# EdwardFerdian/4DFlowNet

Hardware: AMD Instinct MI355X
Metric: 3D patches/sec (train step, patch=24, res×2) (higher is better)
Workload: dtype f32; 1 GPU; cfg2 train_step: patch_size=24 res_increase=2 batch=8/GPU low_resblock=8 hi_resblock=4 fp32; global_batch=8, parallelism=dp1, collective=none

## Files before the change

### 4dflownet_amd/_lib.py

```python
import contextlib
import ctypes
import os

from . import build as _build

_HERE = os.path.dirname(os.path.abspath(__file__))
LIB_PATH = os.path.join(_HERE, "lib4dflow_hip.so")
TEST_LIB_PATH = os.path.join(_HERE, "lib4dflow_hip_test.so")

c_fp = ctypes.c_void_p
c_i = ctypes.c_int
c_i64 = ctypes.c_int64
c_f = ctypes.c_float
c_sz = ctypes.c_size_t

SIGNATURES = {
    "fdn_version": (c_i, []),
    "fdn_last_error": (ctypes.c_char_p, []),
    "fdn_input_features": (c_i, [c_fp] * 8 + [c_i64, c_fp]),
    "fdn_pack_conv64_weights": (c_i, [c_fp, c_fp, c_fp, c_fp]),
    "fdn_conv3d_fwd": (c_i, [c_fp] * 7 + [c_i] * 10 + [c_f, c_i, c_fp]),
    "fdn_conv3d_dgrad": (c_i, [c_fp] * 4 + [c_i] * 10 + [c_fp]),
    "fdn_conv_cout1_dgrad_folded": (c_i, [c_fp, c_fp, c_fp, c_i, c_f, c_fp, c_fp, c_fp, c_sz, c_i, c_i, c_i, c_i, c_i, c_i, c_fp]),
    "fdn_conv_cout1_dgrad_folded_mask": (c_i, [c_fp, c_fp, c_fp, c_i, c_f, c_fp, c_fp, c_fp, c_sz, c_i, c_i, c_i, c_i, c_i, c_i, c_fp]),
    "fdn_fold_halo": (c_i, [c_fp, c_fp, c_fp, c_i, c_fp, c_fp, c_i, c_f, c_fp, c_i, c_i, c_i, c_i, c_i, c_fp]),
    "fdn_conv3d_dgrad_fused": (c_i, [c_fp] * 5 + [c_i, c_f, c_fp, c_i, c_i, c_i, c_i, c_i, c_fp]),
    "fdn_conv64_mask_ok": (c_i, [c_i] * 5),
    "fdn_conv64_fwd_mask": (c_i, [c_fp] * 6 + [c_i] * 5 + [c_f, c_i, c_fp]),
    "fdn_conv64_dgrad_fused_mask": (c_i, [c_fp] * 5 + [c_i, c_f, c_fp, c_i, c_i, c_i, c_i, c_i, c_fp]),
    "fdn_conv64_dgrad_fused_multi": (c_i, [c_fp, c_fp, c_i] + [c_fp] * 4 + [c_i, c_f, c_fp, c_i, c_i, c_i, c_i, c_i, c_fp]),
    "fdn_conv3d_dgrad_fused_part": (c_i, [c_fp] * 5 + [c_i, c_f, c_fp, c_i, c_i, c_i, c_i, c_i, c_i, c_fp]),
    "fdn_fold_halo_border": (c_i, [c_fp, c_fp, c_fp, c_i, c_fp, c_fp, c_i, c_f, c_fp, c_i, c_i, c_i, c_i, c_fp]),
    "fdn_conv1x1_dgrad": (c_i, [c_fp] * 6 + [c_i64, c_fp]),
    "fdn_conv3d_wgrad_workspace_bytes": (c_sz, [c_i] * 7),
    "fdn_conv3d_wgrad_batch_workspace_bytes": (c_sz, [c_i] * 5),
    "fdn_conv3d_wgrad_batch": (c_i, [c_fp, c_fp, c_fp, c_fp, c_i, c_fp, c_sz] + [c_i] * 5 + [c_fp]),
    "fdn_conv3d_wgrad": (c_i, [c_fp] * 6 + [c_sz] + [c_i] * 10 + [c_fp]),
    "fdn_upsample_trilinear_fwd": (c_i, [c_fp, c_fp] + [c_i] * 6 + [c_fp]),
    "fdn_upsample_trilinear_bwd": (c_i, [c_fp, c_fp, c_i, c_f, c_fp] + [c_i] * 6 + [c_fp]),
    "fdn_loss_metrics": (c_i, [c_fp] * 8 + [c_i, c_i64, c_fp]),
    "fdn_loss_metrics_div": (c_i, [c_fp] * 5 + [c_f] + [c_fp] * 3 + [c_i] * 4 + [c_fp]),
    "fdn_gather_patches": (c_i, [c_fp, c_fp, c_i, c_i, c_fp]),
    "fdn_l2_sumsq": (c_i, [c_fp, c_fp, c_i64, c_fp, c_fp]),
    "fdn_adam_step": (c_i, [c_fp] * 5 + [c_i64] + [c_f] * 5 + [c_fp, c_fp, c_fp]),
    "fdn_sum_partials": (c_i, [c_fp, c_i, c_fp, c_fp]),
    "fdn_l2_sumsq_partials": (c_i, [c_fp, c_fp, c_i64, c_fp, c_fp]),
    "fdn_pack_conv64_weights_batch": (c_i, [c_fp, c_fp, c_i, c_fp, c_fp]),
    "fdn_conv64_pack_streams": (c_i, [c_i] * 6),
    "fdn_pack_conv64_weights_batch_streams": (c_i, [c_fp, c_fp, c_i, c_fp, c_i, c_i, c_fp]),
    "fdn_pack_conv64_weights_bf16": (c_i, [c_fp, c_fp, c_fp, c_fp]),
    "fdn_pack_conv64_weights_bf16_batch": (c_i, [c_fp, c_fp, c_i, c_fp, c_fp]),
    "fdn_conv64_fwd_bf16": (c_i, [c_fp] * 5 + [c_i] * 5 + [c_f, c_fp]),
    "fdn_conv64_dgrad_fused_bf16": (c_i, [c_fp] * 5 + [c_i, c_f, c_fp, c_i, c_i, c_i, c_i, c_fp]),
    "fdn_conv64_fwd_bf16_mask": (c_i, [c_fp] * 6 + [c_i] * 5 + [c_f, c_fp]),
    "fdn_conv64_dgrad_fused_bf16_mask": (c_i, [c_fp] * 6 + [c_i, c_f, c_fp, c_i, c_i, c_i, c_i, c_fp]),
    "fdn_conv64_dgrad_fused_bf16_multi": (c_i, [c_fp, c_fp, c_i] + [c_fp] * 4 + [c_i, c_f, c_fp, c_i, c_i, c_i, c_i, c_fp]),
    "fdn_fold_halo_border_bf16": (c_i, [c_fp, c_fp, c_fp, c_i, c_fp, c_fp, c_i, c_f, c_fp, c_i, c_i, c_i, c_i, c_fp]),
    "fdn_input_features_bf16": (c_i, [c_fp] * 8 + [c_i64, c_fp]),
    "fdn_conv3d_fwd_bf16": (c_i, [c_fp] * 7 + [c_i] * 10 + [c_f, c_fp]),
    "fdn_conv3d_wgrad_bf16_workspace_bytes": (c_sz, [c_i] * 7),
    "fdn_conv3d_wgrad_bf16": (c_i, [c_fp] * 6 + [c_sz] + [c_i] * 9 + [c_fp]),
    "fdn_conv3d_wgrad_bf16_batch_workspace_bytes": (c_sz, [c_i] * 5),
    "fdn_conv3d_wgrad_bf16_batch": (c_i, [c_fp, c_fp, c_fp, c_fp, c_i, c_fp, c_sz] + [c_i] * 4 + [c_fp]),
    "fdn_conv_cout1_dgrad_folded_bf16": (c_i, [c_fp, c_fp, c_fp, c_i, c_f, c_fp, c_fp, c_fp, c_sz, c_i, c_i, c_i, c_i, c_i, c_i, c_fp]),
    "fdn_conv_cout1_dgrad_folded_bf16_mask": (c_i, [c_fp, c_fp, c_fp, c_fp, c_i, c_f, c_fp, c_fp, c_fp, c_sz, c_i, c_i, c_i, c_i, c_i, c_i, c_fp]),
    "fdn_conv1x1_dgrad_bf16": (c_i, [c_fp] * 6 + [c_i64, c_fp]),
    "fdn_upsample_trilinear_fwd_bf16": (c_i, [c_fp, c_fp] + [c_i] * 6 + [c_fp]),
    "fdn_upsample_trilinear_bwd_bf16": (c_i, [c_fp, c_fp, c_i, c_f, c_fp] + [c_i] * 6 + [c_fp]),
}


DEBUG_SIGNATURES = {
    "fdn_debug_set_conv64_mt": (c_i, [c_i]),
    "fdn_debug_set_conv64_dbg": (c_i, [c_i]),
    "fdn_debug_set_conv64_shell_slabs": (c_i, [c_i]),
    "fdn_debug_set_conv64_wface_direct": (c_i, [c_i]),
    "fdn_debug_set_conv64_split_dgrad": (c_i, [c_i]),
    "fdn_debug_set_conv64_bf16_mt": (c_i, [c_i]),
    "fdn_debug_set_conv64_bf16_dbg": (c_i, [c_i]),
    "fdn_debug_set_conv64_bf16_mode2": (c_i, [c_i]),
    "fdn_debug_set_heads_mfma": (c_i, [c_i]),
    "fdn_debug_set_upsample_bwd_hb": (c_i, [c_i]),
    "fdn_debug_set_wgrad64_direct": (c_i, [c_i]),
    "fdn_debug_set_conv64_wino_dbg": (c_i, [c_i]),
    "fdn_debug_set_conv64_wino_tile": (c_i, [c_i]),
    "fdn_debug_set_conv64_wino2d_dbg": (c_i, [c_i]),
    "fdn_debug_set_conv64_wino2d_tile": (c_i, [c_i]),
    "fdn_debug_set_conv64_wino2d_variant": (c_i, [c_i]),
    "fdn_debug_set_conv64_wino2d_mb": (c_i, [c_i]),
    "fdn_debug_set_cin3_mfma": (c_i, [c_i]),
    "fdn_debug_set_conv1x1_mfma": (c_i, [c_i]),
    "fdn_debug_set_wgrad64_wino_dbg": (c_i, [c_i]),
    "fdn_debug_set_wgrad64_wino_nodep": (c_i, [c_i]),
    "fdn_debug_set_wgrad64_bf16_dbg": (c_i, [c_i]),
    "fdn_debug_set_wgrad64_bf16_variant": (c_i, [c_i]),
    "fdn_debug_plan_log": (c_i, [c_i]),
    "fdn_debug_plan_read": (c_sz, [ctypes.c_char_p, c_sz]),
}


class FdnError(RuntimeError):
    pass


FDN_VERSION = 161


_product = None
_test = None
_lib = None


def _open(path, sigs, test_hooks=False):
    try:
        built = _build.ensure_built(test_hooks=test_hooks)
    except Exception as e:
        raise FdnError("%s is not usable (%s): %s.  Run `python __graft_entry__.py` or `python 4dflownet_amd/build.py`; "
                       "there is no CPU fallback." % (os.path.basename(path), path, e)) from e
    assert os.path.samefile(built, path)
    lib = ctypes.CDLL(path)
    for name, (res, args) in sigs.items():
        fn = getattr(lib, name)
        fn.restype = res
        fn.argtypes = args
    return lib


def _check_version(lib, path):
    have = lib.fdn_version()
    if have != FDN_VERSION:
        raise FdnError("%s reports fdn_version() = %d, this package mirrors include/fdn.h at FDN_VERSION %d: rebuild (python 4dflownet_amd/build.py)"
                       % (os.path.basename(path), have, FDN_VERSION))
    return lib


def load():
    global _lib, _product
    if _lib is not None:
        return _lib
    if _product is None:
        _product = _check_version(_open(LIB_PATH, SIGNATURES), LIB_PATH)
    _lib = _product
    return _lib


@contextlib.contextmanager
def test_build():
    global _lib, _test
    if _test is None:
        sigs = dict(SIGNATURES)
        sigs.update(DEBUG_SIGNATURES)
        _test = _check_version(_open(TEST_LIB_PATH, sigs, test_hooks=True), TEST_LIB_PATH)
    prev = _lib
    _lib = _test
    try:
        yield _test
    finally:
        _lib = prev


def check(rc, what):
    if rc != 0:
        msg = load().fdn_last_error()
        raise FdnError("%s failed (rc=%d): %s" % (what, rc, msg.decode() if msg else "?"))
```

### 4dflownet_amd/csrc/wgrad64_wino.hip

```cpp
#include "fdn_common.h"
#include <type_traits>

namespace {

struct WgWinoArgs {
    const float* x;
    const float* dz;
    float* partial;
    int N, D, H, W;
    int DT;
    int nth, ntw, ntiles, S;
    unsigned bytes;
    int dbg;
};

FDN_HOOK_VAR(int, fdn_wgrad64_wino_dbg, 0);

constexpr int WTH = 6, WTG = 2, WTW = 4 * WTG;
constexpr int GROWB = 1536;
constexpr int VBYTES = (WTH + 2) * WTG * GROWB;
constexpr int ZBYTES = WTH * WTG * GROWB;
constexpr int WBUFB = VBYTES + ZBYTES;
constexpr int kLocSlot = 5, kXSlot = 6, kZSlot = 13;
constexpr int kLocSlotZ = 10;
constexpr int XSCRATCH = 6 * 4096;
constexpr int ZSCRATCH = 2 * 3072;

template <bool DEP>
__device__ __forceinline__ void wgrad64_wino_body(const WgWinoArgs& p, const int q, char* const smem) {
    constexpr int NP = DEP ? 4 : 3;
    const int tid = threadIdx.x;
    const int lane = tid & 63;
    const int wave = tid >> 6;
    const int li = lane & 31;
    const int kh = lane >> 5;
    const int mq = wave & 1, nq = (wave >> 1) & 1;
    const int eh = wave >> 2;
    const int split = q / NP;
    const int a = q - NP * split;
    const int c16 = tid & 15;
    const int ig = (tid >> 4) & 1;
    const int il = (tid >> 5) & 7;
    const int wave_s = __builtin_amdgcn_readfirstlane(wave);
    const bool xitem = wave_s < 4;
    const bool zitem = wave_s >= 4 && wave_s < 7;
    static_assert(WTH == 6 && WTG == 2, "item-to-wave map above");

    f32x16 acc[3][3];
#pragma unroll
    for (int b = 0; b < 3; ++b)
#pragma unroll
        for (int xp = 0; xp < 3; ++xp)
#pragma unroll
            for (int r = 0; r < 16; ++r) acc[b][xp][r] = 0.f;

    const bool dfast = (FDN_DBG_BITS(p) & 16) != 0;
    const int per_c = p.DT, per_r = p.ntw * per_c, per_n = p.nth * per_r;
    const int per_d = p.nth * p.ntw;
    int tn, td, th, tw;
    int sn, sd, sh, sw;
    if (dfast) {
        int b = split;
        tn = b / per_n; b -= tn * per_n;
        th = b / per_r; b -= th * per_r;
        tw = b / per_c; td = b - tw * per_c;
        b = p.S;
        sn = b / per_n; b -= sn * per_n;
        sh = b / per_r; b -= sh * per_r;
        sw = b / per_c; sd = b - sw * per_c;
    } else {
        int b = split;
        tn = b / per_n; b -= tn * per_n;
        td = b / per_d; b -= td * per_d;
        th = b / p.ntw; tw = b - th * p.ntw;
        b = p.S;
        sn = b / per_n; b -= sn * per_n;
        sd = b / per_d; b -= sd * per_d;
        sh = b / p.ntw; sw = b - sh * p.ntw;
    }
    const int nk = (p.ntiles - split + p.S - 1) / p.S;
    int kload = 0;
    auto advance = [&]() {
        if (kload + 1 < nk) {
            ++kload;
            if (dfast) {
                td += sd; if (td >= p.DT) { td -= p.DT; ++tw; }
                tw += sw; if (tw >= p.ntw) { tw -= p.ntw; ++th; }
                th += sh; if (th >= p.nth) { th -= p.nth; ++tn; }
            } else {
                tw += sw; if (tw >= p.ntw) { tw -= p.ntw; ++th; }
                th += sh; if (th >= p.nth) { th -= p.nth; ++td; }
                td += sd; if (td >= p.DT) { td -= p.DT; ++tn; }
            }
            tn += sn;
        }
    };

    const __amdgpu_buffer_rsrc_t xrs = __builtin_amdgcn_make_buffer_rsrc((void*)p.x, 0, p.bytes, 0x00020000);
    const __amdgpu_buffer_rsrc_t zrs = __builtin_amdgcn_make_buffer_rsrc((void*)p.dz, 0, p.bytes, 0x00020000);
    const fdn_i32x4 xrs_raw = fdn_raw_rsrc(p.x, p.bytes), zrs_raw = fdn_raw_rsrc(p.dz, p.bytes);
    f32x4 raw[6];
    const int wave_u = __builtin_amdgcn_readfirstlane(wave);
    char* const xscr = smem + 3 * WBUFB + wave_u * 1024;
    char* const zscr = smem + 3 * WBUFB + XSCRATCH + (wave_u & 3) * 1024;
    const float sx = a == 1 ? 1.f : -1.f;
    const float cA = a >= 2 ? -1.f : 1.f, cB = 1.f;
    const bool has_zb = DEP && (a == 1 || a == 2);
    unsigned dxb = 0, dzb = 0;
    auto bload = [&](__amdgpu_buffer_rsrc_t r, unsigned vo, unsigned so) {
        return __builtin_bit_cast(f32x4, __builtin_amdgcn_raw_buffer_load_b128(r, (int)vo, (int)so, 0));
    };
    const unsigned tc0 = (unsigned)((il * p.W + 4 * ig) * 256 + c16 * 16);
    unsigned rowoff = 0;
    bool x_in = false, z_in = false;
    unsigned x_so = 0, z_so = 0;
    auto locate = [&]() {
        int qd, zd;
        if (DEP) {
            const int d0 = 2 * td;
            const int pa = a == 0 ? d0 - 1 : d0, pb = a == 3 ? d0 + 2 : d0 + 1;
            qd = min(max(pa, 0), p.D - 1);
            dxb = (unsigned)((min(max(pb, 0), p.D - 1) - qd) * p.H * p.W) * 256u;
            zd = a == 3 ? d0 + 1 : d0;
            dzb = (unsigned)(p.H * p.W) * 256u;
        } else {
            qd = min(max(td + a - 1, 0), p.D - 1);
            zd = td;
        }
        const int h0 = th * WTH - 1, w0 = tw * WTW - 1;
        const unsigned xplane = (unsigned)((tn * p.D + qd) * p.H * p.W) * 256u;
        const unsigned zplane = (unsigned)((tn * p.D + zd) * p.H * p.W) * 256u;
        x_in = __builtin_amdgcn_readfirstlane((int)(h0 >= 0 && h0 + WTH + 2 <= p.H && w0 >= 0 && w0 + WTW + 2 <= p.W)) != 0;
        z_in = __builtin_amdgcn_readfirstlane((int)(h0 + 1 + WTH <= p.H && w0 + 1 + WTW <= p.W)) != 0;
        x_so = xplane + (unsigned)((h0 * p.W + w0) * 256);
        z_so = zplane + (unsigned)(((h0 + 1) * p.W + w0 + 1) * 256);
        if (!x_in && xitem) rowoff = xplane + (unsigned)(min(max(h0 + il, 0), p.H - 1) * p.W * 256 + c16 * 16);
        if (!z_in && zitem) rowoff = h0 + 1 + il < p.H ? zplane + (unsigned)((h0 + 1 + il) * p.W * 256 + c16 * 16) : 0xffffffffu;
    };
    auto load_x = [&](int nn) {
        if (!xitem || (FDN_DBG_BITS(p) & 1)) return;
        const unsigned vo = x_in ? tc0 + (unsigned)(nn * 256) : rowoff + (unsigned)(min(max(tw * WTW + 4 * ig - 1 + nn, 0), p.W - 1) * 256);
        const unsigned so = (unsigned)__builtin_amdgcn_readfirstlane((int)(x_in ? x_so : 0u));
        raw[nn] = bload(xrs, vo, so);
        if (DEP) fdn_lds_dma16_untracked(xrs_raw, fdn_lds_addr(xscr) + (unsigned)(nn * 4096), vo, so + dxb);
    };
    auto load_z = [&](int j) {
        if (!zitem || (FDN_DBG_BITS(p) & 1)) return;
        const int qw = tw * WTW + 4 * ig + j;
        const unsigned vo = z_in ? tc0 + (unsigned)(j * 256) : ((rowoff != 0xffffffffu && qw < p.W) ? rowoff + (unsigned)(qw * 256) : 0xffffffffu);
        const unsigned so = (unsigned)__builtin_amdgcn_readfirstlane((int)(z_in ? z_so : 0u));
        raw[j] = bload(zrs, vo, so);
        if (DEP && has_zb) {
            const unsigned vb = vo == 0xffffffffu ? vo : vo + dzb;
            if (j < 2) raw[4 + j] = bload(zrs, vb, so);
            else fdn_lds_dma16_untracked(zrs_raw, fdn_lds_addr(zscr) + (unsigned)((j - 2) * 3072), vb, so);
        }
    };
    auto combine_x = [&]() {
        if (!DEP || !xitem || (FDN_DBG_BITS(p) & 2)) return;
        asm volatile("s_waitcnt vmcnt(0)" ::: "memory");
#pragma unroll
        for (int nn = 0; nn < 6; ++nn) raw[nn] += sx * *(const f32x4*)(xscr + nn * 4096 + lane * 16);
    };
    auto combine_z = [&]() {
        if (!DEP || !zitem || (FDN_DBG_BITS(p) & 2)) return;
        if (has_zb) asm volatile("s_waitcnt vmcnt(0)" ::: "memory");
#pragma unroll
        for (int j = 0; j < 4; ++j) {
            if (has_zb) raw[j] = cA * raw[j] + cB * (j < 2 ? raw[4 + j] : *(const f32x4*)(zscr + (j - 2) * 3072 + lane * 16));
            else raw[j] = cA * raw[j];
        }
    };
    auto put = [&](char* dst, f32x4 v0, f32x4 v1, f32x4 v2) {
        *(f32x4*)(dst + c16 * 32) = (f32x4){v0.x, v1.x, v0.y, v1.y};
        *(f32x4*)(dst + c16 * 32 + 16) = (f32x4){v0.z, v1.z, v0.w, v1.w};
        *(f32x4*)(dst + 512 + c16 * 16) = v2;
    };
    constexpr float pa = 0.75f, pb = 1.5f, pa2 = 0.5625f, pb2 = 2.25f, pa3 = 0.421875f, pb3 = 3.375f;
    constexpr float pab2 = 1.6875f, pa2b = 0.84375f, ps = 2.8125f, pp = 1.265625f;
    auto write_v = [&](int e, char* buf) {
        if (!xitem || (FDN_DBG_BITS(p) & 2)) return;
        char* dst = buf + (il * WTG + ig) * GROWB + e * 768;
        const f32x4 x0 = raw[0], x1 = raw[1], x2 = raw[2], x3 = raw[3], x4 = raw[4], x5 = raw[5];
        const f32x4 t1 = x4 - pb2 * x2, t2 = pa * x3 - pab2 * x1, t3 = x4 - pa2 * x2, t4 = pb * x3 - pa2b * x1;
        if (e == 0) put(dst, pp * x0 - ps * x2 + x4, t1 - t2, t3 - t4);
        else put(dst, t1 + t2, t3 + t4, pp * x1 - ps * x3 + x5);
    };
    auto write_z = [&](int e, char* buf) {
        if (!zitem || (FDN_DBG_BITS(p) & 2)) return;
        char* dst = buf + VBYTES + (il * WTG + ig) * GROWB + e * 768;
        const f32x4 z0 = raw[0], z1 = raw[1], z2 = raw[2], z3 = raw[3];
        const f32x4 e1 = z0 + pa2 * z2, o1 = pa * z1 + pa3 * z3, e2 = z0 + pb2 * z2, o2 = pb * z1 + pb3 * z3;
        if (e == 0) put(dst, z0, e1 - o1, e2 - o2);
        else put(dst, e1 + o1, e2 + o2, z3);
    };

    locate();
#pragma unroll
    for (int nn = 0; nn < 6; ++nn) load_x(nn);
#pragma unroll
    for (int j = 0; j < 4; ++j) load_z(j);
    combine_x(); combine_z();
#pragma unroll
    for (int e = 0; e < 2; ++e) { write_v(e, smem); write_z(e, smem); }
    advance();
    locate();
#pragma unroll
    for (int nn = 0; nn < 6; ++nn) load_x(nn);
#pragma unroll
    for (int j = 0; j < 4; ++j) load_z(j);
    __syncthreads();

    const int lane_v = kh * GROWB + eh * 768 + (mq * 32 + li) * 8;
    const int lane_z = VBYTES + kh * GROWB + eh * 768 + (nq * 32 + li) * 8;
    const int lane_v1 = kh * GROWB + eh * 768 + 512 + (mq * 32 + li) * 4;
    const int lane_z1 = VBYTES + kh * GROWB + eh * 768 + 512 + (nq * 32 + li) * 4;
    f32x2 Vp[4] = {{1.f, 1.f}, {1.f, 1.f}, {1.f, 1.f}, {1.f, 1.f}}, Zp[2] = {{1.f, 1.f}, {1.f, 1.f}};
    float Vs[4] = {1.f, 1.f, 1.f, 1.f}, Zs[2] = {1.f, 1.f};
    auto issue_v = [&](const char* buf, int line, int slot) {
        if (FDN_DBG_BITS(p) & 4) return;
        Vp[slot] = *(const f32x2*)(buf + lane_v + line * (WTG * GROWB));
        Vs[slot] = *(const float*)(buf + lane_v1 + line * (WTG * GROWB));
    };
    auto issue_z = [&](const char* buf, int line, int slot) {
        if (FDN_DBG_BITS(p) & 4) return;
        Zp[slot] = *(const f32x2*)(buf + lane_z + line * (WTG * GROWB));
        Zs[slot] = *(const float*)(buf + lane_z1 + line * (WTG * GROWB));
    };
    int bcur = 0;
    issue_z(smem, 0, 0);
    issue_v(smem, 0, 0);
    auto tile_loop = [&](auto role) {
    constexpr int ROLE = decltype(role)::value;
#pragma unroll 1
    for (int k = 0; k < nk; ++k) {
        const int bnxt = bcur == 2 ? 0 : bcur + 1;
        const char* cur = smem + bcur * WBUFB;
        char* nxt = smem + bnxt * WBUFB;
#pragma unroll
        for (int s = 0; s < 18; ++s) {
            const int q = s / 3, b = s % 3;
            if (s == 12 && !(FDN_DBG_BITS(p) & 64)) __syncthreads();
            if (s + 1 < 18) {
                const int ln = (s + 1) / 3 + (s + 1) % 3;
                if ((s + 1) % 3 == 2 || s + 1 < 3) issue_v(cur, ln, ln & 3);
                if ((s + 1) % 3 == 0) issue_z(cur, (s + 1) / 3, ((s + 1) / 3) & 1);
            } else {
                issue_v(nxt, 0, 0);
                issue_z(nxt, 0, 0);
            }
            __builtin_amdgcn_sched_barrier(0);
            if (ROLE == 0 && s == 0) combine_x();
            if (ROLE == 1 && s == 2) combine_z();
            if (ROLE == 0 && s < 2) write_v(s, nxt);
            if (ROLE == 1 && s >= 2 && s < 4) write_z(s - 2, nxt);
            if (ROLE == 0 && s == kLocSlot && !(FDN_DBG_BITS(p) & 32)) { advance(); locate(); }
            if (ROLE == 1 && s == kLocSlotZ && !(FDN_DBG_BITS(p) & 32)) { advance(); locate(); }
            if (ROLE == 0 && s >= kXSlot && s < kXSlot + 6) load_x(s - kXSlot);
            if (ROLE == 1 && s >= kZSlot && s < kZSlot + 4) load_z(s - kZSlot);
            acc[b][0] = __builtin_amdgcn_mfma_f32_32x32x2f32(Vp[(q + b) & 3].x, Zp[q & 1].x, acc[b][0], 0, 0, 0);
            acc[b][1] = __builtin_amdgcn_mfma_f32_32x32x2f32(Vp[(q + b) & 3].y, Zp[q & 1].y, acc[b][1], 0, 0, 0);
            acc[b][2] = __builtin_amdgcn_mfma_f32_32x32x2f32(Vs[(q + b) & 3], Zs[q & 1], acc[b][2], 0, 0, 0);
            __builtin_amdgcn_sched_barrier(0);
        }
        bcur = bnxt;
    }
    };
    if (xitem) tile_loop(std::integral_constant<int, 0>{});
    else if (zitem) tile_loop(std::integral_constant<int, 1>{});
    else tile_loop(std::integral_constant<int, 2>{});

    const int lane_e = (int)__builtin_amdgcn_mbcnt_hi(~0u, __builtin_amdgcn_mbcnt_lo(~0u, 0u));
    const int li_e = lane_e & 31, kh_e = lane_e >> 5;
    const int mq_e = wave_s & 1, nq_e = (wave_s >> 1) & 1, eh_e = wave_s >> 2;
    {
        constexpr float c0 = 64.f / 81, ca = -128.f / 243, cb = 32.f / 243;
#pragma unroll
        for (int b = 0; b < 3; ++b) {
            const f32x16 m0 = acc[b][0], m1 = acc[b][1], m2 = acc[b][2];
            if (eh_e == 0) {
                acc[b][0] = c0 * m0 + ca * m1 + cb * m2;
                acc[b][1] = (-pa * ca) * m1 + (-pb * cb) * m2;
                acc[b][2] = (pa2 * ca) * m1 + (pb2 * cb) * m2;
            } else {
                acc[b][0] = ca * m0 + cb * m1;
                acc[b][1] = (pa * ca) * m0 + (pb * cb) * m1;
                acc[b][2] = (pa2 * ca) * m0 + (pb2 * cb) * m1 + m2;
            }
        }
    }
    float* xch = (float*)smem + (size_t)(wave_s & 3) * (5 * 16 * 64) + lane_e;
#pragma unroll
    for (int round = 0; round < 2; ++round) {
        __syncthreads();
        if (eh_e == 1) {
#pragma unroll
            for (int k = 0; k < 9; ++k)
                if ((k < 5) == (round == 0))
#pragma unroll
                    for (int r = 0; r < 16; ++r) xch[((k - 5 * round) * 16 + r) * 64] = acc[k / 3][k % 3][r];
        }
        __syncthreads();
        if (eh_e == 0) {
#pragma unroll
            for (int k = 0; k < 9; ++k)
                if ((k < 5) == (round == 0))
#pragma unroll
                    for (int r = 0; r < 16; ++r) acc[k / 3][k % 3][r] += xch[((k - 5 * round) * 16 + r) * 64];
        }
    }
    if (eh_e == 0) {
        float* out = p.partial + ((size_t)split * (NP * 9) + a * 9) * 4096;
#pragma unroll
        for (int k = 0; k < 9; ++k)
#pragma unroll
            for (int r = 0; r < 16; ++r) {
                const int ci = mq_e * 32 + (r & 3) + 8 * (r >> 2) + 4 * kh_e;
                out[(size_t)k * 4096 + ci * 64 + nq_e * 32 + li_e] = acc[k / 3][k % 3][r];
            }
    }
}

__device__ __forceinline__ int wgrad64_place(int block, int G, bool plain) {
    const int qx = G >> 3, rx = G & 7, xcd = block & 7, j = block >> 3;
    return plain ? block : xcd * qx + min(xcd, rx) + j;
}

template <bool DEP>
__global__ __launch_bounds__(512, 1) void wgrad64_wino_kernel(WgWinoArgs p) {
    extern __shared__ __attribute__((aligned(16))) char smem[];
    wgrad64_wino_body<DEP>(p, wgrad64_place((int)blockIdx.x, (DEP ? 4 : 3) * p.S, (FDN_DBG_BITS(p) & 8) != 0), smem);
}

constexpr int kWgBatchMax = 32;
struct WgWinoBatch {
    WgWinoArgs a;
    const float* x[kWgBatchMax];
    const float* dz[kWgBatchMax];
    int nl;
};
struct WgDwTable { float* dw[kWgBatchMax]; };

template <bool DEP>
__global__ __launch_bounds__(512, 1) void wgrad64_wino_batch_kernel(WgWinoBatch b) {
    extern __shared__ __attribute__((aligned(16))) char smem[];
    constexpr int NP = DEP ? 4 : 3;
    const int per = NP * b.a.S;
    const int qg = wgrad64_place((int)blockIdx.x, per * b.nl, (FDN_DBG_BITS(b.a) & 8) != 0);
    const int layer = qg / per;
    WgWinoArgs p = b.a;
    p.x = b.x[layer]; p.dz = b.dz[layer];
    p.partial = b.a.partial + (size_t)layer * b.a.S * (NP * 9) * 4096;
    wgrad64_wino_body<DEP>(p, qg - layer * per, smem);
}

bool wgrad64_wino_dep_ok(int D) { return D >= 2 && (D & 1) == 0; }
int wgrad64_wino_splits(int N, int D, int H, int W, bool dep) {
    const long long ntiles = (long long)N * (dep ? D / 2 : D) * ((H + WTH - 1) / WTH) * ((W + WTW - 1) / WTW);
    long long S = dep ? 64 : 85;
    if (ntiles < S) S = ntiles > 0 ? ntiles : 1;
    return (int)S;
}

constexpr int kRedParts = 8;
__global__ __launch_bounds__(64 * kRedParts) void wgrad64_reduce_dep_kernel(const float* __restrict__ partial_base, WgDwTable dws, int S) {
    __shared__ f32x4 red[kRedParts - 1][3][64];
    const float* partial = partial_base + (size_t)blockIdx.y * S * 36 * 4096;
    float* dw = dws.dw[blockIdx.y];
    const int col = threadIdx.x & 63, part = threadIdx.x >> 6;
    const int e4 = blockIdx.x * 64 + col;
    const f32x4* p = (const f32x4*)partial + e4;
    const int s0q = (S * part) / kRedParts, s1q = (S * (part + 1)) / kRedParts;
    f32x4 m0 = {0.f, 0.f, 0.f, 0.f}, m1 = m0, m2 = m0, m3 = m0;
    for (int s = s0q; s < s1q; ++s) {
        const f32x4* ps = p + (size_t)s * (36 * 1024);
        m0 += ps[0]; m1 += ps[9 * 1024]; m2 += ps[18 * 1024]; m3 += ps[27 * 1024];
    }
    const f32x4 t0 = m0 + 0.5f * (m1 + m2), t1 = 0.5f * (m1 - m2), t2 = 0.5f * (m1 + m2) + m3;
    if (part) { red[part - 1][0][col] = t0; red[part - 1][1][col] = t1; red[part - 1][2][col] = t2; }
    __syncthreads();
    if (part == 0) {
        f32x4 r0 = t0, r1 = t1, r2 = t2;
#pragma unroll
        for (int q = 0; q < kRedParts - 1; ++q) { r0 += red[q][0][col]; r1 += red[q][1][col]; r2 += red[q][2][col]; }
        ((f32x4*)dw)[e4] = r0;
        ((f32x4*)dw)[9 * 1024 + e4] = r1;
        ((f32x4*)dw)[18 * 1024 + e4] = r2;
    }
}

}

#ifdef FDN_TEST_HOOKS
extern "C" int fdn_debug_set_wgrad64_wino_dbg(int bits) { fdn_wgrad64_wino_dbg = bits; return FDN_OK; }
#endif

FDN_HOOK_VAR(int, fdn_wgrad64_wino_nodep, 0);

size_t fdn_wgrad64_wino_workspace_bytes(int N, int D, int H, int W) {
    const size_t a = (size_t)wgrad64_wino_splits(N, D, H, W, false) * 27, b = wgrad64_wino_dep_ok(D) ? (size_t)wgrad64_wino_splits(N, D, H, W, true) * 36 : 0;
    return (a > b ? a : b) * 4096 * sizeof(float);
}

int fdn_wgrad64_wino_launch(const float* x, const float* dz, float* dw, void* ws, size_t ws_bytes, int N, int D, int H,
                            int W, hipStream_t s, int algo) {
    const bool dep = wgrad64_wino_dep_ok(D) && algo != FDN_ALGO_WINO_W && !fdn_wgrad64_wino_nodep;
    WgWinoArgs a;
    a.x = x; a.dz = dz; a.partial = (float*)ws;
    a.N = N; a.D = D; a.H = H; a.W = W;
    a.DT = dep ? D / 2 : D;
    a.nth = (H + WTH - 1) / WTH; a.ntw = (W + WTW - 1) / WTW;
    a.ntiles = N * a.DT * a.nth * a.ntw;
    a.S = wgrad64_wino_splits(N, D, H, W, dep);
    FDN_REQUIRE((long long)N * D * H * W * 256 < (1ll << 32), "wgrad64: x of %dx%dx%dx%dx64 floats exceeds the 32-bit buffer addressing", N, D, H, W);
    FDN_REQUIRE(ws_bytes >= (size_t)a.S * (dep ? 36 : 27) * 4096 * sizeof(float), "wgrad64 (winograd): workspace too small");
    a.bytes = (unsigned)((long long)N * D * H * W * 256);
    a.dbg = fdn_wgrad64_wino_dbg;
    FDN_PLAN("fam=wgrad_wino op=wgrad dt=f32 N=%d D=%d H=%d W=%d dep=%d splits=%d grid=%d tiles=%d cus=%d", N, D, H, W, dep, a.S, (dep ? 4 : 3) * a.S,
             a.ntiles, fdn_plan_cus());
    if (dep) {
        const size_t lds = (size_t)3 * WBUFB + XSCRATCH + ZSCRATCH;
        if (int rc = fdn_func_max_lds((const void*)wgrad64_wino_kernel<true>, (int)lds, "wgrad64_wino")) return rc;
        hipLaunchKernelGGL(wgrad64_wino_kernel<true>, dim3(4 * a.S), dim3(512), lds, s, a);
        FDN_CHECK_LAUNCH("wgrad64_wino_kernel");
        WgDwTable t;
        t.dw[0] = dw;
        hipLaunchKernelGGL(wgrad64_reduce_dep_kernel, dim3(9 * 1024 / 64), dim3(64 * kRedParts), 0, s, (const float*)ws, t, a.S);
        FDN_CHECK_LAUNCH("wgrad64_reduce_dep_kernel");
        return FDN_OK;
    }
    const size_t lds = (size_t)3 * WBUFB;
    if (int rc = fdn_func_max_lds((const void*)wgrad64_wino_kernel<false>, (int)lds, "wgrad64_wino")) return rc;
    hipLaunchKernelGGL(wgrad64_wino_kernel<false>, dim3(3 * a.S), dim3(512), lds, s, a);
    FDN_CHECK_LAUNCH("wgrad64_wino_kernel");
    return fdn_wgrad64_reduce_launch((const float*)ws, dw, a.S, s);
}

bool fdn_wgrad64_wino_batch_ok(int n_layers, int D, int algo) {
    return n_layers >= 2 && n_layers <= kWgBatchMax && wgrad64_wino_dep_ok(D) && algo != FDN_ALGO_WINO_W && algo != FDN_ALGO_DIRECT && !fdn_wgrad64_wino_nodep;
}
static int wgrad64_wino_batch_splits(int n_layers, int N, int D, int H, int W) {
    const long long ntiles = (long long)N * (D / 2) * ((H + WTH - 1) / WTH) * ((W + WTW - 1) / WTW);
    long long S = 64 / n_layers;
    if (S < 1) S = 1;
    if (ntiles < S) S = ntiles > 0 ? ntiles : 1;
    return (int)S;
}
size_t fdn_wgrad64_wino_batch_workspace_bytes(int n_layers, int N, int D, int H, int W) {
    return (size_t)n_layers * wgrad64_wino_batch_splits(n_layers, N, D, H, W) * 36 * 4096 * sizeof(float);
}
int fdn_wgrad64_wino_batch_launch(const float* const* x, const float* const* dz, float* const* dw, int n_layers, void* ws, size_t ws_bytes,
                                  int N, int D, int H, int W, hipStream_t s) {
    FDN_REQUIRE(fdn_wgrad64_wino_batch_ok(n_layers, D, FDN_ALGO_AUTO), "wgrad64 (batched): %d layers at depth %d are not batchable", n_layers, D);
    FDN_REQUIRE((long long)N * D * H * W * 256 < (1ll << 32), "wgrad64: x of %dx%dx%dx%dx64 floats exceeds the 32-bit buffer addressing", N, D, H, W);
    WgWinoBatch b;
    WgDwTable t;
    b.nl = n_layers;
    for (int i = 0; i < n_layers; ++i) {
        FDN_REQUIRE(x[i] && dz[i] && dw[i], "wgrad64 (batched): NULL pointer for layer %d", i);
        b.x[i] = x[i]; b.dz[i] = dz[i]; t.dw[i] = dw[i];
    }
    WgWinoArgs& a = b.a;
    a.x = nullptr; a.dz = nullptr; a.partial = (float*)ws;
    a.N = N; a.D = D; a.H = H; a.W = W;
    a.DT = D / 2;
    a.nth = (H + WTH - 1) / WTH; a.ntw = (W + WTW - 1) / WTW;
    a.ntiles = N * a.DT * a.nth * a.ntw;
    a.S = wgrad64_wino_batch_splits(n_layers, N, D, H, W);
    FDN_REQUIRE(ws_bytes >= fdn_wgrad64_wino_batch_workspace_bytes(n_layers, N, D, H, W), "wgrad64 (batched): workspace too small");
    a.bytes = (unsigned)((long long)N * D * H * W * 256);
    a.dbg = fdn_wgrad64_wino_dbg;
    FDN_PLAN("fam=wgrad_wino_batch op=wgrad dt=f32 N=%d D=%d H=%d W=%d layers=%d splits=%d grid=%d tiles=%d cus=%d", N, D, H, W, n_layers, a.S,
             4 * a.S * n_layers, a.ntiles, fdn_plan_cus());
    const size_t lds = (size_t)3 * WBUFB + XSCRATCH + ZSCRATCH;
    if (int rc = fdn_func_max_lds((const void*)wgrad64_wino_batch_kernel<true>, (int)lds, "wgrad64_wino_batch")) return rc;
    hipLaunchKernelGGL(wgrad64_wino_batch_kernel<true>, dim3(4 * a.S * n_layers), dim3(512), lds, s, b);
    FDN_CHECK_LAUNCH("wgrad64_wino_batch_kernel");
    hipLaunchKernelGGL(wgrad64_reduce_dep_kernel, dim3(9 * 1024 / 64, n_layers), dim3(64 * kRedParts), 0, s, (const float*)ws, t, a.S);
    FDN_CHECK_LAUNCH("wgrad64_reduce_dep_kernel");
    return FDN_OK;
}

#ifdef FDN_TEST_HOOKS
extern "C" int fdn_debug_set_wgrad64_wino_nodep(int on) { fdn_wgrad64_wino_nodep = on; return FDN_OK; }
#endif
```

Before: 334.3 patches/s.

## Walk wgrad Winograd tiles contiguously per split with depth-innermost order

Replaces the strided tile assignment in the batched Winograd weight-gradient kernel with a contiguous-range walk by default. Each split now owns a consecutive block of tiles ordered n,h,w,d, so successive tiles mostly differ only in depth and the column offsets are recomputed only when the h/w position changes. The tile-advance step moves to the start of the pipelined loop and is done per role, with lane-derived values recomputed inside the loop to shorten live ranges. It also adds a test hook that lists the walk order. The intent is better cache locality across neighbouring depth slices and less per-tile address arithmetic, at the cost of possible load imbalance between splits and a reshuffled prefetch schedule.

```diff
diff --git a/4dflownet_amd/_lib.py b/4dflownet_amd/_lib.py
--- a/4dflownet_amd/_lib.py
+++ b/4dflownet_amd/_lib.py
@@ -92,6 +92,7 @@
     "fdn_debug_set_conv1x1_mfma": (c_i, [c_i]),
     "fdn_debug_set_wgrad64_wino_dbg": (c_i, [c_i]),
     "fdn_debug_set_wgrad64_wino_nodep": (c_i, [c_i]),
+    "fdn_debug_wgrad64_wino_walk": (c_i, [c_i] * 7 + [ctypes.POINTER(c_i), c_i, ctypes.POINTER(c_i)]),
     "fdn_debug_set_wgrad64_bf16_dbg": (c_i, [c_i]),
     "fdn_debug_set_wgrad64_bf16_variant": (c_i, [c_i]),
     "fdn_debug_plan_log": (c_i, [c_i]),
diff --git a/4dflownet_amd/csrc/wgrad64_wino.hip b/4dflownet_amd/csrc/wgrad64_wino.hip
--- a/4dflownet_amd/csrc/wgrad64_wino.hip
+++ b/4dflownet_amd/csrc/wgrad64_wino.hip
@@ -21,16 +21,63 @@
 constexpr int VBYTES = (WTH + 2) * WTG * GROWB;
 constexpr int ZBYTES = WTH * WTG * GROWB;
 constexpr int WBUFB = VBYTES + ZBYTES;
-constexpr int kLocSlot = 5, kXSlot = 6, kZSlot = 13;
-constexpr int kLocSlotZ = 10;
+constexpr int kXSlot = 6, kZSlot = 13;
 constexpr int XSCRATCH = 6 * 4096;
 constexpr int ZSCRATCH = 2 * 3072;
+
+struct WgWalk {
+    int tn, th, tw, td;
+    int sn, sd, sh, sw;
+};
+__host__ __device__ __forceinline__ int wgrad64_walk_first(int s, int T, int S) { return s * (T / S) + (s * (T % S)) / S; }
+__host__ __device__ __forceinline__ int wgrad64_walk_begin(WgWalk& c, int split, int S, int T, int DT, int nth, int ntw, bool stride) {
+    c.sn = c.sd = c.sh = c.sw = 0;
+    if (stride) {
+        const int per_d = nth * ntw, per_n = DT * per_d;
+        int b = split;
+        c.tn = b / per_n; b -= c.tn * per_n;
+        c.td = b / per_d; b -= c.td * per_d;
+        c.th = b / ntw; c.tw = b - c.th * ntw;
+        b = S;
+        c.sn = b / per_n; b -= c.sn * per_n;
+        c.sd = b / per_d; b -= c.sd * per_d;
+        c.sh = b / ntw; c.sw = b - c.sh * ntw;
+        const int nk = split < T ? (T - split + S - 1) / S : 0;
+        return nk;
+    }
+    const int t0 = wgrad64_walk_first(split, T, S), t1 = wgrad64_walk_first(split + 1, T, S);
+    const int per_r = ntw * DT, per_n = nth * per_r;
+    int b = t0;
+    c.tn = b / per_n; b -= c.tn * per_n;
+    c.th = b / per_r; b -= c.th * per_r;
+    c.tw = b / DT; c.td = b - c.tw * DT;
+    return t1 - t0;
+}
+__host__ __device__ __forceinline__ int wgrad64_walk_next(WgWalk& c, bool more, int DT, int nth, int ntw, bool stride) {
+    if (!more) return 0;
+    if (stride) {
+        c.tw += c.sw; if (c.tw >= ntw) { c.tw -= ntw; ++c.th; }
+        c.th += c.sh; if (c.th >= nth) { c.th -= nth; ++c.td; }
+        c.td += c.sd; if (c.td >= DT) { c.td -= DT; ++c.tn; }
+        c.tn += c.sn;
+        return 2;
+    }
+    if (++c.td < DT) return 1;
+    c.td = 0;
+    const bool ww = ++c.tw == ntw;
+    c.tw = ww ? 0 : c.tw;
+    c.th += ww ? 1 : 0;
+    const bool wh = c.th == nth;
+    c.th = wh ? 0 : c.th;
+    c.tn += wh ? 1 : 0;
+    return 2;
+}
 
 template <bool DEP>
 __device__ __forceinline__ void wgrad64_wino_body(const WgWinoArgs& p, const int q, char* const smem) {
     constexpr int NP = DEP ? 4 : 3;
     const int tid = threadIdx.x;
-    const int lane = tid & 63;
+    int lane = tid & 63;
     const int wave = tid >> 6;
     const int li = lane & 31;
     const int kh = lane >> 5;
@@ -38,9 +85,9 @@
     const int eh = wave >> 2;
     const int split = q / NP;
     const int a = q - NP * split;
-    const int c16 = tid & 15;
-    const int ig = (tid >> 4) & 1;
-    const int il = (tid >> 5) & 7;
+    int c16 = tid & 15;
+    int ig = (tid >> 4) & 1;
+    int il = (tid >> 5) & 7;
     const int wave_s = __builtin_amdgcn_readfirstlane(wave);
     const bool xitem = wave_s < 4;
     const bool zitem = wave_s >= 4 && wave_s < 7;
@@ -54,47 +101,9 @@
 #pragma unroll
             for (int r = 0; r < 16; ++r) acc[b][xp][r] = 0.f;
 
-    const bool dfast = (FDN_DBG_BITS(p) & 16) != 0;
-    const int per_c = p.DT, per_r = p.ntw * per_c, per_n = p.nth * per_r;
-    const int per_d = p.nth * p.ntw;
-    int tn, td, th, tw;
-    int sn, sd, sh, sw;
-    if (dfast) {
-        int b = split;
-        tn = b / per_n; b -= tn * per_n;
-        th = b / per_r; b -= th * per_r;
-        tw = b / per_c; td = b - tw * per_c;
-        b = p.S;
-        sn = b / per_n; b -= sn * per_n;
-        sh = b / per_r; b -= sh * per_r;
-        sw = b / per_c; sd = b - sw * per_c;
-    } else {
-        int b = split;
-        tn = b / per_n; b -= tn * per_n;
-        td = b / per_d; b -= td * per_d;
-        th = b / p.ntw; tw = b - th * p.ntw;
-        b = p.S;
-        sn = b / per_n; b -= sn * per_n;
-        sd = b / per_d; b -= sd * per_d;
-        sh = b / p.ntw; sw = b - sh * p.ntw;
-    }
-    const int nk = (p.ntiles - split + p.S - 1) / p.S;
-    int kload = 0;
-    auto advance = [&]() {
-        if (kload + 1 < nk) {
-            ++kload;
-            if (dfast) {
-                td += sd; if (td >= p.DT) { td -= p.DT; ++tw; }
-                tw += sw; if (tw >= p.ntw) { tw -= p.ntw; ++th; }
-                th += sh; if (th >= p.nth) { th -= p.nth; ++tn; }
-            } else {
-                tw += sw; if (tw >= p.ntw) { tw -= p.ntw; ++th; }
-                th += sh; if (th >= p.nth) { th -= p.nth; ++td; }
-                td += sd; if (td >= p.DT) { td -= p.DT; ++tn; }
-            }
-            tn += sn;
-        }
-    };
+    const bool stride = (FDN_DBG_BITS(p) & 16) != 0;
+    WgWalk wk;
+    const int nk = wgrad64_walk_begin(wk, split, p.S, p.ntiles, p.DT, p.nth, p.ntw, stride);
 
     const __amdgpu_buffer_rsrc_t xrs = __builtin_amdgcn_make_buffer_rsrc((void*)p.x, 0, p.bytes, 0x00020000);
     const __amdgpu_buffer_rsrc_t zrs = __builtin_amdgcn_make_buffer_rsrc((void*)p.dz, 0, p.bytes, 0x00020000);
@@ -105,48 +114,61 @@
     char* const zscr = smem + 3 * WBUFB + XSCRATCH + (wave_u & 3) * 1024;
     const float sx = a == 1 ? 1.f : -1.f;
     const float cA = a >= 2 ? -1.f : 1.f, cB = 1.f;
-    const bool has_zb = DEP && (a == 1 || a == 2);
+    bool has_zb = DEP && (a == 1 || a == 2);
     unsigned dxb = 0, dzb = 0;
     auto bload = [&](__amdgpu_buffer_rsrc_t r, unsigned vo, unsigned so) {
         return __builtin_bit_cast(f32x4, __builtin_amdgcn_raw_buffer_load_b128(r, (int)vo, (int)so, 0));
     };
-    const unsigned tc0 = (unsigned)((il * p.W + 4 * ig) * 256 + c16 * 16);
+    unsigned tc0 = (unsigned)((il * p.W + 4 * ig) * 256 + c16 * 16);
     unsigned rowoff = 0;
     bool x_in = false, z_in = false;
     unsigned x_so = 0, z_so = 0;
+    unsigned x_col = 0, z_col = 0;
+    auto locate_col = [&]() {
+        const int h0 = wk.th * WTH - 1, w0 = wk.tw * WTW - 1;
+        x_in = __builtin_amdgcn_readfirstlane((int)(h0 >= 0 && h0 + WTH + 2 <= p.H && w0 >= 0 && w0 + WTW + 2 <= p.W)) != 0;
+        z_in = __builtin_amdgcn_readfirstlane((int)(h0 + 1 + WTH <= p.H && w0 + 1 + WTW <= p.W)) != 0;
+        x_col = (unsigned)((h0 * p.W + w0) * 256);
+        z_col = (unsigned)(((h0 + 1) * p.W + w0 + 1) * 256);
+    };
     auto locate = [&]() {
         int qd, zd;
         if (DEP) {
-            const int d0 = 2 * td;
+            const int d0 = 2 * wk.td;
             const int pa = a == 0 ? d0 - 1 : d0, pb = a == 3 ? d0 + 2 : d0 + 1;
             qd = min(max(pa, 0), p.D - 1);
             dxb = (unsigned)((min(max(pb, 0), p.D - 1) - qd) * p.H * p.W) * 256u;
             zd = a == 3 ? d0 + 1 : d0;
             dzb = (unsigned)(p.H * p.W) * 256u;
         } else {
-            qd = min(max(td + a - 1, 0), p.D - 1);
-            zd = td;
-        }
-        const int h0 = th * WTH - 1, w0 = tw * WTW - 1;
-        const unsigned xplane = (unsigned)((tn * p.D + qd) * p.H * p.W) * 256u;
-        const unsigned zplane = (unsigned)((tn * p.D + zd) * p.H * p.W) * 256u;
-        x_in = __builtin_amdgcn_readfirstlane((int)(h0 >= 0 && h0 + WTH + 2 <= p.H && w0 >= 0 && w0 + WTW + 2 <= p.W)) != 0;
-        z_in = __builtin_amdgcn_readfirstlane((int)(h0 + 1 + WTH <= p.H && w0 + 1 + WTW <= p.W)) != 0;
-        x_so = xplane + (unsigned)((h0 * p.W + w0) * 256);
-        z_so = zplane + (unsigned)(((h0 + 1) * p.W + w0 + 1) * 256);
+            qd = min(max(wk.td + a - 1, 0), p.D - 1);
+            zd = wk.td;
+        }
+        const unsigned xplane = (unsigned)((wk.tn * p.D + qd) * p.H * p.W) * 256u;
+        const unsigned zplane = (unsigned)((wk.tn * p.D + zd) * p.H * p.W) * 256u;
+        x_so = xplane + x_col;
+        z_so = zplane + z_col;
+        const int h0 = wk.th * WTH - 1;
         if (!x_in && xitem) rowoff = xplane + (unsigned)(min(max(h0 + il, 0), p.H - 1) * p.W * 256 + c16 * 16);
         if (!z_in && zitem) rowoff = h0 + 1 + il < p.H ? zplane + (unsigned)((h0 + 1 + il) * p.W * 256 + c16 * 16) : 0xffffffffu;
     };
+    auto step = [&](bool more) {
+        const int moved = wgrad64_walk_next(wk, more, p.DT, p.nth, p.ntw, stride);
+        wk.tn = __builtin_amdgcn_readfirstlane(wk.tn); wk.th = __builtin_amdgcn_readfirstlane(wk.th);
+        wk.tw = __builtin_amdgcn_readfirstlane(wk.tw); wk.td = __builtin_amdgcn_readfirstlane(wk.td);
+        if (moved == 2) locate_col();
+        locate();
+    };
     auto load_x = [&](int nn) {
         if (!xitem || (FDN_DBG_BITS(p) & 1)) return;
-        const unsigned vo = x_in ? tc0 + (unsigned)(nn * 256) : rowoff + (unsigned)(min(max(tw * WTW + 4 * ig - 1 + nn, 0), p.W - 1) * 256);
+        const unsigned vo = x_in ? tc0 + (unsigned)(nn * 256) : rowoff + (unsigned)(min(max(wk.tw * WTW + 4 * ig - 1 + nn, 0), p.W - 1) * 256);
         const unsigned so = (unsigned)__builtin_amdgcn_readfirstlane((int)(x_in ? x_so : 0u));
         raw[nn] = bload(xrs, vo, so);
         if (DEP) fdn_lds_dma16_untracked(xrs_raw, fdn_lds_addr(xscr) + (unsigned)(nn * 4096), vo, so + dxb);
     };
     auto load_z = [&](int j) {
         if (!zitem || (FDN_DBG_BITS(p) & 1)) return;
-        const int qw = tw * WTW + 4 * ig + j;
+        const int qw = wk.tw * WTW + 4 * ig + j;
         const unsigned vo = z_in ? tc0 + (unsigned)(j * 256) : ((rowoff != 0xffffffffu && qw < p.W) ? rowoff + (unsigned)(qw * 256) : 0xffffffffu);
         const unsigned so = (unsigned)__builtin_amdgcn_readfirstlane((int)(z_in ? z_so : 0u));
         raw[j] = bload(zrs, vo, so);
@@ -195,6 +217,7 @@
         else put(dst, e1 + o1, e2 + o2, z3);
     };
 
+    locate_col();
     locate();
 #pragma unroll
     for (int nn = 0; nn < 6; ++nn) load_x(nn);
@@ -203,18 +226,17 @@
     combine_x(); combine_z();
 #pragma unroll
     for (int e = 0; e < 2; ++e) { write_v(e, smem); write_z(e, smem); }
-    advance();
-    locate();
+    step(1 < nk);
 #pragma unroll
     for (int nn = 0; nn < 6; ++nn) load_x(nn);
 #pragma unroll
     for (int j = 0; j < 4; ++j) load_z(j);
     __syncthreads();
 
-    const int lane_v = kh * GROWB + eh * 768 + (mq * 32 + li) * 8;
-    const int lane_z = VBYTES + kh * GROWB + eh * 768 + (nq * 32 + li) * 8;
-    const int lane_v1 = kh * GROWB + eh * 768 + 512 + (mq * 32 + li) * 4;
-    const int lane_z1 = VBYTES + kh * GROWB + eh * 768 + 512 + (nq * 32 + li) * 4;
+    int lane_v = kh * GROWB + eh * 768 + (mq * 32 + li) * 8;
+    int lane_z = VBYTES + kh * GROWB + eh * 768 + (nq * 32 + li) * 8;
+    int lane_v1 = kh * GROWB + eh * 768 + 512 + (mq * 32 + li) * 4;
+    int lane_z1 = VBYTES + kh * GROWB + eh * 768 + 512 + (nq * 32 + li) * 4;
     f32x2 Vp[4] = {{1.f, 1.f}, {1.f, 1.f}, {1.f, 1.f}, {1.f, 1.f}}, Zp[2] = {{1.f, 1.f}, {1.f, 1.f}};
     float Vs[4] = {1.f, 1.f, 1.f, 1.f}, Zs[2] = {1.f, 1.f};
     auto issue_v = [&](const char* buf, int line, int slot) {
@@ -232,8 +254,25 @@
     issue_v(smem, 0, 0);
     auto tile_loop = [&](auto role) {
     constexpr int ROLE = decltype(role)::value;
+    {
+        const int t = wave_s * 64 + (int)__builtin_amdgcn_mbcnt_hi(~0u, __builtin_amdgcn_mbcnt_lo(~0u, 0u));
+        lane = t & 63; c16 = t & 15; ig = (t >> 4) & 1; il = (t >> 5) & 7;
+        tc0 = (unsigned)((il * p.W + 4 * ig) * 256 + c16 * 16);
+        const int li_r = t & 31, kh_r = (t >> 5) & 1;
+        const int mq_r = wave_s & 1, nq_r = (wave_s >> 1) & 1, eh_r = wave_s >> 2;
+        lane_v = kh_r * GROWB + eh_r * 768 + (mq_r * 32 + li_r) * 8;
+        lane_z = VBYTES + kh_r * GROWB + eh_r * 768 + (nq_r * 32 + li_r) * 8;
+        lane_v1 = kh_r * GROWB + eh_r * 768 + 512 + (mq_r * 32 + li_r) * 4;
+        lane_z1 = VBYTES + kh_r * GROWB + eh_r * 768 + 512 + (nq_r * 32 + li_r) * 4;
+        locate_col();
+        int a_r = a;
+        asm volatile("" : "+s"(a_r));
+        has_zb = DEP && (a_r == 1 || a_r == 2);
+    }
+    if (ROLE == 1 && !(FDN_DBG_BITS(p) & 32)) step(2 < nk);
+    int k = 0;
 #pragma unroll 1
-    for (int k = 0; k < nk; ++k) {
+    do {
         const int bnxt = bcur == 2 ? 0 : bcur + 1;
         const char* cur = smem + bcur * WBUFB;
         char* nxt = smem + bnxt * WBUFB;
@@ -250,12 +289,11 @@
                 issue_z(nxt, 0, 0);
             }
             __builtin_amdgcn_sched_barrier(0);
+            if (ROLE == 0 && s == 0 && !(FDN_DBG_BITS(p) & 32)) step(k + 2 < nk);
             if (ROLE == 0 && s == 0) combine_x();
             if (ROLE == 1 && s == 2) combine_z();
             if (ROLE == 0 && s < 2) write_v(s, nxt);
             if (ROLE == 1 && s >= 2 && s < 4) write_z(s - 2, nxt);
-            if (ROLE == 0 && s == kLocSlot && !(FDN_DBG_BITS(p) & 32)) { advance(); locate(); }
-            if (ROLE == 1 && s == kLocSlotZ && !(FDN_DBG_BITS(p) & 32)) { advance(); locate(); }
             if (ROLE == 0 && s >= kXSlot && s < kXSlot + 6) load_x(s - kXSlot);
             if (ROLE == 1 && s >= kZSlot && s < kZSlot + 4) load_z(s - kZSlot);
             acc[b][0] = __builtin_amdgcn_mfma_f32_32x32x2f32(Vp[(q + b) & 3].x, Zp[q & 1].x, acc[b][0], 0, 0, 0);
@@ -263,8 +301,9 @@
             acc[b][2] = __builtin_amdgcn_mfma_f32_32x32x2f32(Vs[(q + b) & 3], Zs[q & 1], acc[b][2], 0, 0, 0);
             __builtin_amdgcn_sched_barrier(0);
         }
+        if (ROLE == 1 && !(FDN_DBG_BITS(p) & 32)) step(k + 3 < nk);
         bcur = bnxt;
-    }
+    } while (++k < nk);
     };
     if (xitem) tile_loop(std::integral_constant<int, 0>{});
     else if (zitem) tile_loop(std::integral_constant<int, 1>{});
@@ -483,4 +522,20 @@
 
 #ifdef FDN_TEST_HOOKS
 extern "C" int fdn_debug_set_wgrad64_wino_nodep(int on) { fdn_wgrad64_wino_nodep = on; return FDN_OK; }
+extern "C" int fdn_debug_wgrad64_wino_walk(int N, int D, int H, int W, int layers, int dep, int split, int* seq, int cap, int* splits) {
+    if (N < 1 || D < 1 || H < 1 || W < 1 || layers < 1 || (dep && !wgrad64_wino_dep_ok(D)) || (layers > 1 && !fdn_wgrad64_wino_batch_ok(layers, D, dep ? FDN_ALGO_AUTO : FDN_ALGO_WINO_W)))
+        return -1;
+    const int DT = dep ? D / 2 : D, nth = (H + WTH - 1) / WTH, ntw = (W + WTW - 1) / WTW, T = N * DT * nth * ntw;
+    const int S = layers > 1 ? wgrad64_wino_batch_splits(layers, N, D, H, W) : wgrad64_wino_splits(N, D, H, W, dep != 0);
+    if (splits) *splits = S;
+    if (split < 0 || split >= S) return -1;
+    const bool stride = (fdn_wgrad64_wino_dbg & 16) != 0;
+    WgWalk c;
+    const int nk = wgrad64_walk_begin(c, split, S, T, DT, nth, ntw, stride);
+    for (int k = 0; k < nk; ++k) {
+        if (k < cap && seq) { seq[4 * k] = c.tn; seq[4 * k + 1] = c.td; seq[4 * k + 2] = c.th; seq[4 * k + 3] = c.tw; }
+        wgrad64_walk_next(c, k + 1 < nk, DT, nth, ntw, stride);
+    }
+    return nk;
+}
 #endif
```

Result: no change. 335.5 patches/s (median of 6 runs) (+0.3%).
